# adalca/neurite

Measured on AMD Instinct MI355X. Metric: Mvoxels/sec interpn+Dice on 160^3 x 32-label, higher is better.
Workload: dtype f32

## Files before the change

neurite_amd/csrc/fused_wc.h:

```cpp

#pragma once

#include <type_traits>

#include "dice_reduce.h"
#include "interpn_core.h"

namespace {

#ifndef WC_NST_WARP
#define WC_NST_WARP 3
#endif
#ifndef WC_NST_FUSED
#define WC_NST_FUSED 2
#endif
#ifndef WC_NST_BWD
#define WC_NST_BWD 3
#endif
constexpr int WC_SLOTS = 128;
constexpr int WC_OVF = 16;
constexpr int WC_TRASH_ROW = WC_SLOTS + WC_OVF;
constexpr int WC_ROWS = WC_TRASH_ROW + 1;
constexpr unsigned WC_NOROW = 0x01ffffffu;
constexpr unsigned WC_TAGS_OFF = WC_ROWS * 128;
constexpr unsigned WC_LIST_OFF = WC_TAGS_OFF + 528;
constexpr unsigned WC_BC_OFF = WC_LIST_OFF + 512;
constexpr unsigned WC_WAVE_BYTES = WC_BC_OFF + 128;
constexpr unsigned WC_BLOCK_BYTES = 4 * WC_WAVE_BYTES;
static_assert(WC_LIST_OFF % 16 == 0 && WC_BC_OFF % 16 == 0 && WC_WAVE_BYTES % 16 == 0, "LDS layout");
static_assert((WC_SLOTS + 1) * 4 <= 528 && WC_ROWS <= 256, "LDS layout");
static_assert(2 * WC_BLOCK_BYTES <= 160 * 1024, "two blocks per CU");

typedef __attribute__((address_space(3))) char wc_lds_char;
typedef __attribute__((address_space(3))) nrt_f4 wc_lds_f4;
typedef __attribute__((address_space(3))) volatile nrt_i4 wc_lds_vi4;
typedef __attribute__((address_space(3))) volatile unsigned wc_lds_vu32;
typedef unsigned wc_u3 __attribute__((ext_vector_type(3)));
typedef unsigned wc_u4 __attribute__((ext_vector_type(4)));
typedef float wc_f3 __attribute__((ext_vector_type(3)));

__device__ __forceinline__ void wc_corner(float pv, float mx, int &i0, int &i1, float &w0) {
    const float cl = fminf(fmaxf(pv, 0.0f), mx);
    const float l0 = floorf(cl);
    const float l1 = fminf(nrt_add(l0, 1.0f), mx);
    i0 = (int)l0; i1 = (int)l1;
    w0 = nrt_sub(l1, cl);
}

__device__ __forceinline__ __amdgpu_buffer_rsrc_t wc_rsrc(const void *base, unsigned bytes) {
    const unsigned long long v = (unsigned long long)base;
    const void *u = (const void *)(((unsigned long long)(unsigned)__builtin_amdgcn_readfirstlane((unsigned)(v >> 32)) << 32) |
                                   (unsigned long long)(unsigned)__builtin_amdgcn_readfirstlane((unsigned)v));
    return __builtin_amdgcn_make_buffer_rsrc((void *)u, 0, __builtin_amdgcn_readfirstlane((int)bytes), 0x00020000);
}

struct WcBwd {
    const float *sums, *gdice;
    float eps;
    float *gloc;
};

template <int MODE, bool STORE, bool MM, bool FILL, bool DICE, int BWD = 0>
__device__ __forceinline__ void wc_item(const InterpArgs &a, const TileGeom &tg, const float *__restrict__ fixed, float *__restrict__ fpart,
                                        float *__restrict__ mpart, const XmWork &xw, char *wc_smem, const WcBwd &bw = WcBwd{nullptr, nullptr, 0.0f, nullptr}) {
    constexpr int G = 8, L = 32;
    static_assert(BWD == 0 || (DICE && !STORE && !MM), "the backward form reads a second row per voxel and stores the location gradient only");
    const int b = __builtin_amdgcn_readfirstlane(xw.b);
    const unsigned prow = (unsigned)__builtin_amdgcn_readfirstlane((int)xw.prow), ucol = (unsigned)__builtin_amdgcn_readfirstlane((int)xw.ucol);
    const unsigned RY = 1u << tg.lry, RZ = 1u << tg.lrz;
    const unsigned nRz = (tg.nTz + RZ - 1) / RZ;
    const unsigned reg = ucol / (RY * RZ), wr = ucol % (RY * RZ);
    const unsigned cy = (reg / nRz) * RY + wr / RZ, cz = (reg % nRz) * RZ + wr % RZ;
    const int x0 = __builtin_amdgcn_readfirstlane(xw.x0), y0 = (int)cy << 2, z0 = (int)cz << 3;
    int npass = __builtin_amdgcn_readfirstlane(xw.xlen);
    if (cy >= tg.nTy || cz >= tg.nTz || npass < 0) npass = 0;

    const int lane = threadIdx.x & 63, wave = threadIdx.x >> 6;
    const int g = lane >> 3, p = lane & 7;
    const int dzt = (0x1320 >> ((g & 3) * 4)) & 15;
    const int yy = y0 + 2 * (wave >> 1) + (g >> 2), zz = z0 + 4 * (wave & 1) + dzt;
    const bool yzvalid = (yy < a.O[1]) && (zz < a.O[2]);
    const int yc = min(yy, a.O[1] - 1), zc = min(zz, a.O[2] - 1);
    const unsigned qyz = (unsigned)yc * (unsigned)a.O[2] + (unsigned)zc, qstep = (unsigned)a.O[1] * (unsigned)a.O[2];
    const unsigned SY = (unsigned)a.S[1], SZ = (unsigned)a.S[2];
    const float mxx = (float)(a.S[0] - 1), mxy = (float)(a.S[1] - 1), mxz = (float)(a.S[2] - 1);
    const float fyc = (float)yc, fzc = (float)zc;
    const float ly = (yc == 0) ? 0.0f : ((yc == a.O[1] - 1) ? mxy : nrt_mul(a.delta[1], fyc));
    const float lz = (zc == 0) ? 0.0f : ((zc == a.O[2] - 1) ? mxz : nrt_mul(a.delta[2], fzc));

    const char *volb = (const char *)a.vol + (long long)b * a.vol_bs * 4ll;
    const unsigned long long volbytes = (unsigned long long)a.S[0] * SY * SZ * 128ull;
    const unsigned outbytes = a.nout * 128u;
    const __amdgpu_buffer_rsrc_t vres = wc_rsrc(volb, (unsigned)volbytes);
    const __amdgpu_buffer_rsrc_t lres = wc_rsrc(MODE != NRT_LOC_LINSPACE ? (const char *)(a.loc + (long long)b * a.loc_bs) : volb, a.nout * 12u);
    const __amdgpu_buffer_rsrc_t fres = wc_rsrc(DICE ? (const char *)fixed + (long long)b * a.out_bs * 4ll : volb, outbytes);
    const __amdgpu_buffer_rsrc_t ores = wc_rsrc(STORE ? (const char *)a.out + (long long)b * a.out_bs * 4ll : volb, outbytes);
    const __amdgpu_buffer_rsrc_t gres = wc_rsrc(BWD ? (const char *)(bw.gloc + (long long)b * a.nout * 3) : volb, a.nout * 12u);
    const unsigned gl_lane = (p == 0 && yzvalid) ? qyz * 12u : 0xffffffffu;
    float ca[4] = {0.0f, 0.0f, 0.0f, 0.0f}, cb[4] = {0.0f, 0.0f, 0.0f, 0.0f};
    if (BWD == 1) {
        const float *sm = bw.sums + (long long)b * 3 * L;
#pragma unroll
        for (int k = 0; k < 4; ++k) {
            const int l = p * 4 + k;
            const float num = 2.0f * sm[l] + bw.eps, den = sm[L + l] + sm[2 * L + l] + bw.eps;
            const float gd = bw.gdice[(long long)b * L + l];
            if (den != 0.0f) { ca[k] = 2.0f * gd / den; cb[k] = -2.0f * gd * num / (den * den); }
        }
    }
    const unsigned loc_lane = qyz * 12u, row_lane = (qyz * 8u + (unsigned)p) * 16u;
    const unsigned out_lane = yzvalid ? row_lane : 0xffffffffu;
    const unsigned loc_step = qstep * 12u, row_step = qstep * 128u;
    const unsigned p16 = (unsigned)p * 16u;

    wc_lds_char *wl = (wc_lds_char *)wc_smem + wave * WC_WAVE_BYTES;
    wc_lds_vu32 *tags = (wc_lds_vu32 *)(wl + WC_TAGS_OFF);
    wc_lds_char *lrow = wl + p * 16;
    tags[lane] = ~0u;
    tags[lane + 64] = ~0u;
    const bool cx1 = (p & 4) != 0, cy1 = (p & 2) != 0, cz1 = (p & 1) != 0;

    nrt_f2 stp_l = {0, 0}, stp_h = {0, 0}, stt_l = {0, 0}, stt_h = {0, 0}, spp_l = {0, 0}, spp_h = {0, 0};
    float mnt = INFINITY, mxt = -INFINITY, mnp = INFINITY, mxp = -INFINITY;

    struct Pass {
        float w0x, w0y, w0z;
        unsigned sl[8];
        unsigned lr[4], ld[4];
        unsigned xr[4], xd[4];
        int n;
        int xq;
        float mk[3];
        bool oob;
        nrt_f4 T;
        nrt_f4 F[4], Fx[4];
        float pn[3];
    };
    struct Mg { float w0x, w0y, w0z; bool oob, miss; unsigned rid, slot, t1, t2, mytag; float mk[3]; };
    constexpr int NST = ((BWD ? WC_NST_BWD : (DICE ? WC_NST_FUSED : WC_NST_WARP)) > 2) ? 3 : 2;
    constexpr bool XSH = NST == 3 && DICE;
    Pass A, B, C;
    nrt_f4 FxS[4] = {{0.f, 0.f, 0.f, 0.f}, {0.f, 0.f, 0.f, 0.f}, {0.f, 0.f, 0.f, 0.f}, {0.f, 0.f, 0.f, 0.f}};
    auto reset = [&](Pass &s) {
        s.w0x = s.w0y = s.w0z = 0.f; s.n = 0; s.xq = x0; s.oob = false; s.mk[0] = s.mk[1] = s.mk[2] = 0.f;
        s.T = (nrt_f4){0.f, 0.f, 0.f, 0.f};
#pragma unroll
        for (int i = 0; i < 4; ++i) { s.F[i] = s.Fx[i] = (nrt_f4){0.f, 0.f, 0.f, 0.f}; s.lr[i] = s.xr[i] = WC_NOROW << 7; s.ld[i] = s.xd[i] = WC_TRASH_ROW * 128u; }
#pragma unroll
        for (int i = 0; i < 8; ++i) s.sl[i] = 0;
        s.pn[0] = s.pn[1] = s.pn[2] = 0.f;
    };
    reset(A); reset(B);
    if (NST == 3) reset(C);

    auto fetch_loc = [&](int pass, Pass &s) {
        if (MODE != NRT_LOC_LINSPACE) {
            const wc_u3 v = __builtin_bit_cast(wc_u3, __builtin_amdgcn_raw_buffer_load_b96(lres, loc_lane, (unsigned)(x0 + pass) * loc_step, 0));
            s.pn[0] = __uint_as_float(v[0]); s.pn[1] = __uint_as_float(v[1]); s.pn[2] = __uint_as_float(v[2]);
        }
    };
    auto fetch_row = [&](unsigned rowoff) -> nrt_f4 {
        return __builtin_bit_cast(nrt_f4, __builtin_amdgcn_raw_buffer_load_b128(vres, rowoff | p16, 0, 0));
    };

    auto m1a = [&](int pass, const Pass &s, Mg &m) {
        const int xq = x0 + pass;
        float px, py, pz;
        if (MODE == NRT_LOC_ABSOLUTE) { px = s.pn[0]; py = s.pn[1]; pz = s.pn[2]; }
        else if (MODE == NRT_LOC_SHIFT) { px = nrt_add((float)xq, s.pn[0]); py = nrt_add(fyc, s.pn[1]); pz = nrt_add(fzc, s.pn[2]); }
        else { px = (xq == 0) ? 0.0f : ((xq == a.O[0] - 1) ? mxx : nrt_mul(a.delta[0], (float)xq)); py = ly; pz = lz; }
        int i0x, i1x, i0y, i1y, i0z, i1z;
        wc_corner(px, mxx, i0x, i1x, m.w0x);
        wc_corner(py, mxy, i0y, i1y, m.w0y);
        wc_corner(pz, mxz, i0z, i1z, m.w0z);
        m.oob = FILL ? ((px < 0.0f) || (px > mxx) || (py < 0.0f) || (py > mxy) || (pz < 0.0f) || (pz > mxz)) : false;
        if (BWD) {
            m.mk[0] = (fminf(fmaxf(px, 0.0f), mxx) == px) ? 1.0f : 0.0f;
            m.mk[1] = (fminf(fmaxf(py, 0.0f), mxy) == py) ? 1.0f : 0.0f;
            m.mk[2] = (fminf(fmaxf(pz, 0.0f), mxz) == pz) ? 1.0f : 0.0f;
        }
        const unsigned ix = cx1 ? i1x : i0x, iy = cy1 ? i1y : i0y, iz = cz1 ? i1z : i0z;
        m.rid = nrt_mad24(nrt_mad24(ix, SY, iy), SZ, iz);
        m.slot = ((ix & 3u) << 5) | ((iy & 3u) << 3) | (iz & 7u);
        m.mytag = (m.rid << 6) | (unsigned)lane;
        m.t1 = tags[m.slot];
    };
    auto m1b = [&](Mg &m) {
        m.miss = (m.t1 ^ m.mytag) >= 64u;
        tags[m.miss ? m.slot : (unsigned)WC_SLOTS] = m.mytag;
        m.t2 = tags[m.slot];
    };
    auto m1c = [&](int pass, const Mg &m, Pass &s) {
        const unsigned x2 = m.t2 ^ m.mytag;
        const bool served = x2 < 64u;
        const bool loader = m.miss && x2 == 0u;
        const bool orphan = !served;
        const unsigned long long Ml = __builtin_amdgcn_ballot_w64(loader), Mo = __builtin_amdgcn_ballot_w64(orphan);
        const unsigned long long Mf = Ml | Mo;
        const int no = __builtin_popcountll(Mo);
        int n = __builtin_popcountll(Mf);
        const unsigned ro = __builtin_amdgcn_mbcnt_hi((unsigned)(Mo >> 32), __builtin_amdgcn_mbcnt_lo((unsigned)Mo, 0u));
        const unsigned rf = __builtin_amdgcn_mbcnt_hi((unsigned)(Mf >> 32), __builtin_amdgcn_mbcnt_lo((unsigned)Mf, 0u));
        bool fetcher = loader || orphan;
        unsigned src = orphan ? (unsigned)WC_SLOTS + ro : m.slot;
        unsigned e = fetcher ? rf : (unsigned)n + ((unsigned)lane - rf);
        if (__builtin_expect(no > WC_OVF, 0)) {
            tags[lane] = ~0u;
            tags[lane + 64] = ~0u;
            e = (unsigned)lane; fetcher = true; src = (unsigned)lane; n = 64;
        }
        const unsigned src128 = src * 128u;
        const unsigned tp = ((e & 7u) << 3) | (e >> 3);
        typedef unsigned wc_u2 __attribute__((ext_vector_type(2)));
        *(__attribute__((address_space(3))) volatile wc_u2 *)(wl + WC_LIST_OFF + tp * 8u) =
            (wc_u2){fetcher ? (m.rid << 7) : (WC_NOROW << 7), fetcher ? src128 : (unsigned)WC_TRASH_ROW * 128u};
        ((__attribute__((address_space(3))) volatile unsigned short *)(wl + WC_BC_OFF))[lane] = (unsigned short)src128;
        const nrt_i4 la = *(wc_lds_vi4 *)(wl + WC_LIST_OFF + g * 64), lb = *(wc_lds_vi4 *)(wl + WC_LIST_OFF + g * 64 + 16);
        const nrt_i4 sh = *(wc_lds_vi4 *)(wl + WC_BC_OFF + g * 16);
        s.lr[0] = (unsigned)la[0]; s.ld[0] = (unsigned)la[1]; s.lr[1] = (unsigned)la[2]; s.ld[1] = (unsigned)la[3];
        s.lr[2] = (unsigned)lb[0]; s.ld[2] = (unsigned)lb[1]; s.lr[3] = (unsigned)lb[2]; s.ld[3] = (unsigned)lb[3];
        if (__builtin_expect(n > 32, 0)) {
            const nrt_i4 lc = *(wc_lds_vi4 *)(wl + WC_LIST_OFF + g * 64 + 32), le = *(wc_lds_vi4 *)(wl + WC_LIST_OFF + g * 64 + 48);
            s.xr[0] = (unsigned)lc[0]; s.xd[0] = (unsigned)lc[1]; s.xr[1] = (unsigned)lc[2]; s.xd[1] = (unsigned)lc[3];
            s.xr[2] = (unsigned)le[0]; s.xd[2] = (unsigned)le[1]; s.xr[3] = (unsigned)le[2]; s.xd[3] = (unsigned)le[3];
        }
#pragma unroll
        for (int c = 0; c < 4; ++c) { s.sl[2 * c] = (unsigned)sh[c] & 0xffffu; s.sl[2 * c + 1] = (unsigned)sh[c] >> 16; }
        s.w0x = m.w0x; s.w0y = m.w0y; s.w0z = m.w0z; s.oob = m.oob; s.n = n;
        if (BWD) { s.mk[0] = m.mk[0]; s.mk[1] = m.mk[1]; s.mk[2] = m.mk[2]; }
        s.xq = x0 + pass;
    };
    auto issue = [&](Pass &s) {
#pragma unroll
        for (int i = 0; i < 4; ++i) s.F[i] = fetch_row(s.lr[i]);
        if (!XSH && __builtin_expect(s.n > 32, 0)) {
#pragma unroll
            for (int i = 0; i < 4; ++i) s.Fx[i] = fetch_row(s.xr[i]);
        }
        if (DICE) s.T = __builtin_bit_cast(nrt_f4, __builtin_amdgcn_raw_buffer_load_b128(fres, row_lane, (unsigned)s.xq * row_step, 2));
    };
    auto issue_x = [&](Pass &s) {
        if (XSH && __builtin_expect(s.n > 32, 0)) {
#pragma unroll
            for (int i = 0; i < 4; ++i) FxS[i] = fetch_row(s.xr[i]);
        }
    };
    auto deliver = [&](Pass &s) {
#pragma unroll
        for (int i = 0; i < 4; ++i) *(wc_lds_f4 *)(lrow + s.ld[i]) = s.F[i];
        if (__builtin_expect(s.n > 32, 0)) {
#pragma unroll
            for (int i = 0; i < 4; ++i) *(wc_lds_f4 *)(lrow + s.xd[i]) = XSH ? FxS[i] : s.Fx[i];
        }
    };

    const int last = npass - 1;
    auto step = [&](int pass, Pass &s, Pass &o, Pass &nx, auto masked) {
        constexpr bool MASKED = decltype(masked)::value;
        issue(o);
        __builtin_amdgcn_sched_barrier(0);
        deliver(s);
        nrt_f4 R[8];
#pragma unroll
        for (int corner = 0; corner < 8; ++corner) R[corner] = *(const wc_lds_f4 *)(lrow + s.sl[corner]);
        __builtin_amdgcn_sched_barrier(0);
        Mg m;
        m1a(min(pass + NST, last), s, m);
        __builtin_amdgcn_sched_barrier(0);
        const float w1x = nrt_sub(1.0f, s.w0x), w1y = nrt_sub(1.0f, s.w0y), w1z = nrt_sub(1.0f, s.w0z);
        const nrt_f2 wy2 = {s.w0y, w1y}, wz2 = {s.w0z, w1z};
        const nrt_f2 wxy0 = (nrt_f2){s.w0x, s.w0x} * wy2, wxy1 = (nrt_f2){w1x, w1x} * wy2;
        nrt_f2 wt2[4];
        wt2[0] = (nrt_f2){wxy0[0], wxy0[0]} * wz2;
        wt2[1] = (nrt_f2){wxy0[1], wxy0[1]} * wz2;
        wt2[2] = (nrt_f2){wxy1[0], wxy1[0]} * wz2;
        wt2[3] = (nrt_f2){wxy1[1], wxy1[1]} * wz2;
        nrt_f2 al = {0.0f, 0.0f}, ah = {0.0f, 0.0f};
        constexpr bool BLEND = BWD != 2;
#pragma unroll
        for (int corner = 0; corner < (BLEND ? 4 : 0); ++corner) {
            const float wt = wt2[corner >> 1][corner & 1];
            const nrt_f2 w2 = {wt, wt};
            al = al + w2 * (nrt_f2){R[corner][0], R[corner][1]};
            ah = ah + w2 * (nrt_f2){R[corner][2], R[corner][3]};
        }
        asm volatile("" : "+v"(al), "+v"(ah));
        __builtin_amdgcn_sched_barrier(0);
        m1b(m);
        __builtin_amdgcn_sched_barrier(0);
#pragma unroll
        for (int corner = 4; corner < (BLEND ? 8 : 4); ++corner) {
            const float wt = wt2[corner >> 1][corner & 1];
            const nrt_f2 w2 = {wt, wt};
            al = al + w2 * (nrt_f2){R[corner][0], R[corner][1]};
            ah = ah + w2 * (nrt_f2){R[corner][2], R[corner][3]};
        }
        nrt_f4 acc = {al[0], al[1], ah[0], ah[1]};
        const unsigned xqcur = (unsigned)s.xq;
        const float cw0x = s.w0x, cw0y = s.w0y, cw0z = s.w0z, cmx = s.mk[0], cmy = s.mk[1], cmz = s.mk[2];
        const bool coob = s.oob;
        if (!BWD) {
            if (FILL) {
#pragma unroll
                for (int c = 0; c < 4; ++c) acc[c] = apply_fill(acc[c], s.oob, a.fill_f);
            }
            if (STORE) __builtin_amdgcn_raw_buffer_store_b128(__builtin_bit_cast(wc_u4, acc), ores, out_lane, (unsigned)s.xq * row_step, 2);
        }
        const nrt_f4 Tcur = s.T;
        asm volatile("" : "+v"(acc));
        __builtin_amdgcn_sched_barrier(0);
        m1c(min(pass + NST, last), m, s);
        __builtin_amdgcn_sched_barrier(0);
        if (BWD) {
            nrt_f2 gl2 = {Tcur[0], Tcur[1]}, gh2 = {Tcur[2], Tcur[3]};
            if (BWD == 1) {
                gl2 = __builtin_elementwise_fma((nrt_f2){cb[0], cb[1]}, (nrt_f2){acc[0], acc[1]}, (nrt_f2){ca[0], ca[1]} * gl2);
                gh2 = __builtin_elementwise_fma((nrt_f2){cb[2], cb[3]}, (nrt_f2){acc[2], acc[3]}, (nrt_f2){ca[2], ca[3]} * gh2);
            }
            if (FILL && coob) { gl2 = (nrt_f2){0.0f, 0.0f}; gh2 = gl2; }
            float gacc[3];
            loc_grad_rows(R, gl2, gh2, cw0x, w1x, cw0y, w1y, cw0z, w1z, cmx, cmy, cmz, gacc);
#pragma unroll
            for (int d = 0; d < 3; ++d) {
                float r = gacc[d];
                r += __int_as_float(__builtin_amdgcn_update_dpp(0, __float_as_int(r), 0xB1, 0xF, 0xF, true));
                r += __int_as_float(__builtin_amdgcn_update_dpp(0, __float_as_int(r), 0x4E, 0xF, 0xF, true));
                r += __int_as_float(__builtin_amdgcn_update_dpp(0, __float_as_int(r), 0x141, 0xF, 0xF, true));
                gacc[d] = r;
            }
            __builtin_amdgcn_raw_buffer_store_b96(__builtin_bit_cast(wc_u3, (wc_f3){gacc[0], gacc[1], gacc[2]}), gres, gl_lane, xqcur * loc_step, 0);
        } else if (DICE) {
            nrt_f4 T = Tcur;
            if (MASKED) {
#pragma unroll
                for (int c = 0; c < 4; ++c) { T[c] = yzvalid ? T[c] : 0.0f; acc[c] = yzvalid ? acc[c] : 0.0f; }
            }
            const nrt_f2 pl = {acc[0], acc[1]}, ph = {acc[2], acc[3]}, tl = {T[0], T[1]}, th = {T[2], T[3]};
            stp_l = stp_l + tl * pl; stp_h = stp_h + th * ph;
            stt_l = stt_l + tl * tl; stt_h = stt_h + th * th;
            spp_l = spp_l + pl * pl; spp_h = spp_h + ph * ph;
            if (MM) {
                if (!MASKED || yzvalid) {
#pragma unroll
                    for (int c = 0; c < 4; ++c) {
                        mnt = fminf(mnt, Tcur[c]); mxt = fmaxf(mxt, Tcur[c]);
                        mnp = fminf(mnp, acc[c]); mxp = fmaxf(mxp, acc[c]);
                    }
                }
            }
        }
        if (DICE && !BWD) asm volatile("" : "+v"(stp_l), "+v"(stp_h), "+v"(stt_l), "+v"(stt_h), "+v"(spp_l), "+v"(spp_h));
        else asm volatile("" :: "v"(acc));
        __builtin_amdgcn_sched_barrier(0);
        fetch_loc(min(pass + 2 * NST, last), s);
        issue_x(nx);
        __builtin_amdgcn_sched_barrier(0);
    };
    auto march = [&](auto masked) {
        Mg m;
        if constexpr (NST == 3) {
            fetch_loc(0, A);
            fetch_loc(min(1, last), B);
            fetch_loc(min(2, last), C);
            m1a(0, A, m); m1b(m); m1c(0, m, A);
            issue(A);
            fetch_loc(min(3, last), A);
            m1a(min(1, last), B, m); m1b(m); m1c(min(1, last), m, B);
            issue(B);
            fetch_loc(min(4, last), B);
            m1a(min(2, last), C, m); m1b(m); m1c(min(2, last), m, C);
            fetch_loc(min(5, last), C);
            issue_x(A);
            __builtin_amdgcn_sched_barrier(0);
            int pass = 0;
            for (; pass + 2 < npass; pass += 3) {
                step(pass, A, C, B, masked);
                step(pass + 1, B, A, C, masked);
                step(pass + 2, C, B, A, masked);
            }
            if (pass < npass) step(pass, A, C, B, masked);
            if (pass + 1 < npass) step(pass + 1, B, A, C, masked);
            return;
        }
        fetch_loc(0, A);
        fetch_loc(min(1, last), B);
        m1a(0, A, m); m1b(m); m1c(0, m, A);
        issue(A);
        fetch_loc(min(2, last), A);
        m1a(min(1, last), B, m); m1b(m); m1c(min(1, last), m, B);
        fetch_loc(min(3, last), B);
        __builtin_amdgcn_sched_barrier(0);
        int pass = 0;
        for (; pass + 1 < npass; pass += 2) {
            step(pass, A, B, B, masked);
            step(pass + 1, B, A, A, masked);
        }
        if (pass < npass) step(pass, A, B, B, masked);
    };
    if (npass > 0) {
        if (DICE && !BWD && __builtin_amdgcn_ballot_w64(!yzvalid) != 0ull) march(std::true_type());
        else march(std::false_type());
    }

    if (!DICE || BWD) return;
    nrt_f4 stp = {stp_l[0], stp_l[1], stp_h[0], stp_h[1]}, stt = {stt_l[0], stt_l[1], stt_h[0], stt_h[1]},
           spp = {spp_l[0], spp_l[1], spp_h[0], spp_h[1]};
#pragma unroll
    for (int c = 0; c < 4; ++c) {
        stp[c] = wave_xor_add(stp[c], G);
        stt[c] = wave_xor_add(stt[c], G);
        spp[c] = wave_xor_add(spp[c], G);
    }
    for (int off = 1; off < NRT_WAVE; off <<= 1) {
        mnt = fminf(mnt, __shfl_xor(mnt, off, NRT_WAVE)); mxt = fmaxf(mxt, __shfl_xor(mxt, off, NRT_WAVE));
        mnp = fminf(mnp, __shfl_xor(mnp, off, NRT_WAVE)); mxp = fmaxf(mxp, __shfl_xor(mxp, off, NRT_WAVE));
    }
    __syncthreads();
    float (*red)[3 * L + 4] = (float (*)[3 * L + 4])wc_smem;
    if (lane < G) {
#pragma unroll
        for (int c = 0; c < 4; ++c) {
            red[wave][0 * L + 4 * lane + c] = stp[c];
            red[wave][1 * L + 4 * lane + c] = stt[c];
            red[wave][2 * L + 4 * lane + c] = spp[c];
        }
    }
    if (lane == 0) { red[wave][3 * L + 0] = mnt; red[wave][3 * L + 1] = mxt; red[wave][3 * L + 2] = mnp; red[wave][3 * L + 3] = mxp; }
    __syncthreads();
    const long long pbase = (long long)b * tg.prows + prow;
    for (int i = threadIdx.x; i < 3 * L; i += 256) {
        float s = red[0][i];
#pragma unroll
        for (int w2 = 1; w2 < 4; ++w2) s += red[w2][i];
        fpart[pbase * 3 * L + i] = s;
    }
    if (threadIdx.x < 4) {
        float m = red[0][3 * L + threadIdx.x];
        for (int w2 = 1; w2 < 4; ++w2)
            m = (threadIdx.x & 1) ? fmaxf(m, red[w2][3 * L + threadIdx.x]) : fminf(m, red[w2][3 * L + threadIdx.x]);
        mpart[pbase * 4 + threadIdx.x] = m;
    }
    xmarch_zero_rows(tg, xw, 3 * L, fpart, mpart);
}


template <typename ITEM>
__device__ __forceinline__ void wc_persistent_loop(const TileGeom &tg, int O0, unsigned *__restrict__ queue, ITEM item) {
    __shared__ unsigned s_next[2];
    const unsigned home = blockIdx.x % NRT_NXCD;
    for (;;) {
        __syncthreads();
        if (threadIdx.x == 0) {
            unsigned kk = home, jb = 0xffffffffu;
            for (unsigned t = 0; t < NRT_NXCD; ++t) {
                const unsigned q = (home + t) % NRT_NXCD;
                const unsigned v = atomicAdd(&queue[q * 16u], 1u);
                if (v < tg.items_x) { kk = q; jb = v; break; }
            }
            s_next[0] = kk; s_next[1] = jb;
        }
        __syncthreads();
        const unsigned kk = s_next[0], jb = s_next[1];
        if (jb == 0xffffffffu) break;
        XmWork xw;
        if (!xmarch_work_at(tg, O0, kk, jb, xw)) continue;
        item(xw);
    }
    if (threadIdx.x == 0 && atomicAdd(&queue[NRT_NXCD * 16u], 1u) == gridDim.x - 1) {
        for (unsigned q = 0; q <= NRT_NXCD; ++q) queue[q * 16u] = 0u;
    }
}

template <int MODE, bool STORE, bool MM, bool FILL, bool DICE = true, bool PERSIST = false>
__global__ __launch_bounds__(256, 2) void warp_dice_wc(InterpArgs a, TileGeom tg, const float *__restrict__ fixed,
                                                        float *__restrict__ fpart, float *__restrict__ mpart, unsigned *__restrict__ queue) {
    extern __shared__ __attribute__((aligned(16))) char wc_smem[];
    if (!PERSIST) {
        XmWork xw;
        if (!xmarch_work(tg, a.O[0], xw)) return;
        wc_item<MODE, STORE, MM, FILL, DICE>(a, tg, fixed, fpart, mpart, xw, wc_smem);
        return;
    }
    wc_persistent_loop(tg, a.O[0], queue, [&](const XmWork &xw) { wc_item<MODE, STORE, MM, FILL, DICE>(a, tg, fixed, fpart, mpart, xw, wc_smem); });
}

template <int MODE, bool FILL, int BWD, bool PERSIST>
__global__ __launch_bounds__(256, 2) void warp_dice_wc_bwd(InterpArgs a, TileGeom tg, const float *__restrict__ rows, WcBwd bw,
                                                            unsigned *__restrict__ queue) {
    extern __shared__ __attribute__((aligned(16))) char wc_smem[];
    if (!PERSIST) {
        XmWork xw;
        if (!xmarch_work(tg, a.O[0], xw)) return;
        wc_item<MODE, false, false, FILL, true, BWD>(a, tg, rows, nullptr, nullptr, xw, wc_smem, bw);
        return;
    }
    wc_persistent_loop(tg, a.O[0], queue, [&](const XmWork &xw) { wc_item<MODE, false, false, FILL, true, BWD>(a, tg, rows, nullptr, nullptr, xw, wc_smem, bw); });
}

inline bool wc_persistent(const TileGeom &tg) { return NRT_NXCD * tg.items_x > 2u * (unsigned)nrt_num_cus(); }
static_assert(NRT_RING_GATHER_OFF == 0 && (NRT_NXCD + 1) * 16 <= NRT_RING_CCE_OFF, "the work counters of a launch stay in the gather's words of a slot");

template <int MODE, bool STORE, bool MM, bool FILL>
int launch_wc_inst(const InterpArgs &a, const TileGeom &tg, unsigned nblocks, int batch, const float *fixed, float *fpart, float *mpart,
                   hipStream_t st) {
    const unsigned items = NRT_NXCD * tg.items_x, slots = 2u * (unsigned)nrt_num_cus();
    unsigned *queue = wc_persistent(tg) ? nrt_ring_slot(st) : nullptr;
    if (queue) {
        if (hipFuncSetAttribute((const void *)warp_dice_wc<MODE, STORE, MM, FILL, true, true>, hipFuncAttributeMaxDynamicSharedMemorySize,
                                (int)WC_BLOCK_BYTES) != hipSuccess)
            return NRT_ERR_LAUNCH;
        hipLaunchKernelGGL((warp_dice_wc<MODE, STORE, MM, FILL, true, true>), dim3(nrt_xcd_grid(slots)), dim3(256), WC_BLOCK_BYTES, st, a, tg, fixed,
                           fpart, mpart, queue);
        return NRT_OK;
    }
    if (hipFuncSetAttribute((const void *)warp_dice_wc<MODE, STORE, MM, FILL>, hipFuncAttributeMaxDynamicSharedMemorySize, (int)WC_BLOCK_BYTES) != hipSuccess)
        return NRT_ERR_LAUNCH;
    hipLaunchKernelGGL((warp_dice_wc<MODE, STORE, MM, FILL>), dim3(items), dim3(256), WC_BLOCK_BYTES, st, a, tg, fixed, fpart, mpart,
                       (unsigned *)nullptr);
    (void)nblocks; (void)batch;
    return NRT_OK;
}

template <int MODE, bool FILL>
int launch_wc_fill(const InterpArgs &a, const TileGeom &tg, unsigned nblocks, int batch, bool store, bool minmax, const float *fixed,
                   float *fpart, float *mpart, hipStream_t st) {
    if (store) return minmax ? launch_wc_inst<MODE, true, true, FILL>(a, tg, nblocks, batch, fixed, fpart, mpart, st)
                             : launch_wc_inst<MODE, true, false, FILL>(a, tg, nblocks, batch, fixed, fpart, mpart, st);
    return minmax ? launch_wc_inst<MODE, false, true, FILL>(a, tg, nblocks, batch, fixed, fpart, mpart, st)
                  : launch_wc_inst<MODE, false, false, FILL>(a, tg, nblocks, batch, fixed, fpart, mpart, st);
}

template <int MODE>
int launch_wc_mode(const InterpArgs &a, const TileGeom &tg, unsigned nblocks, int batch, bool store, bool minmax, const float *fixed,
                   float *fpart, float *mpart, hipStream_t st) {
    return a.has_fill ? launch_wc_fill<MODE, true>(a, tg, nblocks, batch, store, minmax, fixed, fpart, mpart, st)
                      : launch_wc_fill<MODE, false>(a, tg, nblocks, batch, store, minmax, fixed, fpart, mpart, st);
}

inline bool wc_applies(const TileGeom &tg, int G, const InterpArgs &a) {
    return tg.x_march && G == 8 && tg.lty == 2 && tg.ltz == 3 && !tg.plane_major &&
           (unsigned long long)a.S[0] * a.S[1] * a.S[2] * 128ull < 0xffffff00ull;
}

inline int launch_wc(const InterpArgs &a, const TileGeom &tg, unsigned nblocks, int batch, int mode, bool store, bool minmax,
                     const float *fixed, float *fpart, float *mpart, hipStream_t st) {
    switch (mode) {
        case NRT_LOC_ABSOLUTE: return launch_wc_mode<NRT_LOC_ABSOLUTE>(a, tg, nblocks, batch, store, minmax, fixed, fpart, mpart, st);
        case NRT_LOC_SHIFT: return launch_wc_mode<NRT_LOC_SHIFT>(a, tg, nblocks, batch, store, minmax, fixed, fpart, mpart, st);
        default: return launch_wc_mode<NRT_LOC_LINSPACE>(a, tg, nblocks, batch, store, minmax, fixed, fpart, mpart, st);
    }
}

template <int MODE, bool FILL>
int launch_wc_interpn_inst(const InterpArgs &a, const TileGeom &tg, hipStream_t st) {
    const unsigned items = NRT_NXCD * tg.items_x, slots = 2u * (unsigned)nrt_num_cus();
    unsigned *queue = (items > slots) ? nrt_ring_slot(st) : nullptr;
    if (queue) {
        if (hipFuncSetAttribute((const void *)warp_dice_wc<MODE, true, false, FILL, false, true>, hipFuncAttributeMaxDynamicSharedMemorySize,
                                (int)WC_BLOCK_BYTES) != hipSuccess)
            return NRT_ERR_LAUNCH;
        hipLaunchKernelGGL((warp_dice_wc<MODE, true, false, FILL, false, true>), dim3(nrt_xcd_grid(slots)), dim3(256), WC_BLOCK_BYTES, st, a, tg,
                           (const float *)nullptr, (float *)nullptr, (float *)nullptr, queue);
        return NRT_OK;
    }
    if (hipFuncSetAttribute((const void *)warp_dice_wc<MODE, true, false, FILL, false>, hipFuncAttributeMaxDynamicSharedMemorySize,
                            (int)WC_BLOCK_BYTES) != hipSuccess)
        return NRT_ERR_LAUNCH;
    hipLaunchKernelGGL((warp_dice_wc<MODE, true, false, FILL, false>), dim3(items), dim3(256), WC_BLOCK_BYTES, st, a, tg, (const float *)nullptr,
                       (float *)nullptr, (float *)nullptr, (unsigned *)nullptr);
    return NRT_OK;
}

template <int MODE, bool FILL, int BWD>
int launch_wc_bwd_inst(const InterpArgs &a, const TileGeom &tg, const float *rows, const WcBwd &bw, hipStream_t st) {
    const unsigned items = NRT_NXCD * tg.items_x, slots = 2u * (unsigned)nrt_num_cus();
    unsigned *queue = (items > slots) ? nrt_ring_slot(st) : nullptr;
    if (queue) {
        if (hipFuncSetAttribute((const void *)warp_dice_wc_bwd<MODE, FILL, BWD, true>, hipFuncAttributeMaxDynamicSharedMemorySize, (int)WC_BLOCK_BYTES) != hipSuccess)
            return NRT_ERR_LAUNCH;
        hipLaunchKernelGGL((warp_dice_wc_bwd<MODE, FILL, BWD, true>), dim3(nrt_xcd_grid(slots)), dim3(256), WC_BLOCK_BYTES, st, a, tg, rows, bw, queue);
        return NRT_OK;
    }
    if (hipFuncSetAttribute((const void *)warp_dice_wc_bwd<MODE, FILL, BWD, false>, hipFuncAttributeMaxDynamicSharedMemorySize, (int)WC_BLOCK_BYTES) != hipSuccess)
        return NRT_ERR_LAUNCH;
    hipLaunchKernelGGL((warp_dice_wc_bwd<MODE, FILL, BWD, false>), dim3(items), dim3(256), WC_BLOCK_BYTES, st, a, tg, rows, bw, (unsigned *)nullptr);
    return NRT_OK;
}

template <int MODE, bool FILL>
int launch_wc_bwd_mode(const InterpArgs &a, const TileGeom &tg, const float *rows, const WcBwd &bw, hipStream_t st) {
    return bw.sums ? launch_wc_bwd_inst<MODE, FILL, 1>(a, tg, rows, bw, st) : launch_wc_bwd_inst<MODE, FILL, 2>(a, tg, rows, bw, st);
}

}

int nrt_wc_bwd_launch(const void *args, int batch, int mode, const float *rows, const float *sums, const float *grad_dice, float eps,
                      float *grad_loc, void *stream) {
    const InterpArgs &a = *(const InterpArgs *)args;
    if (mode != NRT_LOC_ABSOLUTE && mode != NRT_LOC_SHIFT) return NRT_ERR_INVALID_ARG;
    TileGeom tg;
    unsigned nblocks, grid;
    const int t = xmarch_default_tune();
    tile_geometry(a.O, 8, t, t, tg, nblocks);
    xmarch_setup_mixed(a.O, batch, t, tg, grid);
    hipStream_t st = nrt_stream(stream);
    const WcBwd bw = {sums, grad_dice, eps, grad_loc};
    int rc;
    if (mode == NRT_LOC_ABSOLUTE) rc = a.has_fill ? launch_wc_bwd_mode<NRT_LOC_ABSOLUTE, true>(a, tg, rows, bw, st) : launch_wc_bwd_mode<NRT_LOC_ABSOLUTE, false>(a, tg, rows, bw, st);
    else rc = a.has_fill ? launch_wc_bwd_mode<NRT_LOC_SHIFT, true>(a, tg, rows, bw, st) : launch_wc_bwd_mode<NRT_LOC_SHIFT, false>(a, tg, rows, bw, st);
    if (rc != NRT_OK) return rc;
    NRT_CHECK_LAUNCH();
    return NRT_OK;
}

bool nrt_wc_interpn_supported(const void *args, int batch) {
    const InterpArgs &a = *(const InterpArgs *)args;
    if (a.C != 32 || !xmarch_applies(a.O, batch)) return false;
    if ((unsigned long long)a.nout * 128ull >= (1ull << 32)) return false;
    if ((long long)a.S[0] * a.S[1] >= (1 << 24) || a.S[2] >= (1 << 24) || (long long)a.O[0] * a.O[1] >= (1 << 24) || a.O[2] >= (1 << 24)) return false;
    TileGeom tg;
    unsigned nblocks, grid;
    const int t = xmarch_default_tune();
    tile_geometry(a.O, 8, t, t, tg, nblocks);
    xmarch_setup_mixed(a.O, batch, t, tg, grid);
    return wc_applies(tg, 8, a);
}

int nrt_wc_interpn_launch(const void *args, int batch, int mode, void *stream) {
    const InterpArgs &a = *(const InterpArgs *)args;
    TileGeom tg;
    unsigned nblocks, grid;
    const int t = xmarch_default_tune();
    tile_geometry(a.O, 8, t, t, tg, nblocks);
    xmarch_setup_mixed(a.O, batch, t, tg, grid);
    hipStream_t st = nrt_stream(stream);
    int rc;
    switch (mode) {
        case NRT_LOC_ABSOLUTE: rc = a.has_fill ? launch_wc_interpn_inst<NRT_LOC_ABSOLUTE, true>(a, tg, st) : launch_wc_interpn_inst<NRT_LOC_ABSOLUTE, false>(a, tg, st); break;
        case NRT_LOC_SHIFT: rc = a.has_fill ? launch_wc_interpn_inst<NRT_LOC_SHIFT, true>(a, tg, st) : launch_wc_interpn_inst<NRT_LOC_SHIFT, false>(a, tg, st); break;
        default: rc = a.has_fill ? launch_wc_interpn_inst<NRT_LOC_LINSPACE, true>(a, tg, st) : launch_wc_interpn_inst<NRT_LOC_LINSPACE, false>(a, tg, st); break;
    }
    if (rc != NRT_OK) return rc;
    NRT_CHECK_LAUNCH();
    return NRT_OK;
}
```

Before: 19770.

## Shrink always-fetched row groups to three and skip unused row stores

Makes the number of always-issued row fetch groups configurable (default still 4). Row fetches and LDS deliveries beyond the live count are skipped using a wave-uniform count, taken with readfirstlane. The first loop iteration is peeled out of the three-stage and two-stage march loops. The aim is to cut wasted LDS writes and fetches when few unique rows are needed and to give the scheduler a steady-state loop, at the cost of extra branching and larger code.

```diff
diff --git a/neurite_amd/csrc/fused_wc.h b/neurite_amd/csrc/fused_wc.h
--- a/neurite_amd/csrc/fused_wc.h
+++ b/neurite_amd/csrc/fused_wc.h
@@ -16,6 +16,9 @@
 #endif
 #ifndef WC_NST_BWD
 #define WC_NST_BWD 3
+#endif
+#ifndef WC_FIXED_GROUPS
+#define WC_FIXED_GROUPS 4
 #endif
 constexpr int WC_SLOTS = 128;
 constexpr int WC_OVF = 16;
@@ -123,29 +126,35 @@
     nrt_f2 stp_l = {0, 0}, stp_h = {0, 0}, stt_l = {0, 0}, stt_h = {0, 0}, spp_l = {0, 0}, spp_h = {0, 0};
     float mnt = INFINITY, mxt = -INFINITY, mnp = INFINITY, mxp = -INFINITY;
 
+    constexpr int FG = WC_FIXED_GROUPS, NX = 8 - FG;
+    static_assert(FG == 3 || FG == 4, "WC_FIXED_GROUPS");
     struct Pass {
         float w0x, w0y, w0z;
         unsigned sl[8];
-        unsigned lr[4], ld[4];
-        unsigned xr[4], xd[4];
+        unsigned lr[FG], ld[FG];
+        unsigned xr[NX], xd[NX];
         int n;
         int xq;
         float mk[3];
         bool oob;
         nrt_f4 T;
-        nrt_f4 F[4], Fx[4];
+        nrt_f4 F[FG], Fx[NX];
         float pn[3];
     };
     struct Mg { float w0x, w0y, w0z; bool oob, miss; unsigned rid, slot, t1, t2, mytag; float mk[3]; };
     constexpr int NST = ((BWD ? WC_NST_BWD : (DICE ? WC_NST_FUSED : WC_NST_WARP)) > 2) ? 3 : 2;
     constexpr bool XSH = NST == 3 && DICE;
     Pass A, B, C;
-    nrt_f4 FxS[4] = {{0.f, 0.f, 0.f, 0.f}, {0.f, 0.f, 0.f, 0.f}, {0.f, 0.f, 0.f, 0.f}, {0.f, 0.f, 0.f, 0.f}};
+    nrt_f4 FxS[NX];
+#pragma unroll
+    for (int i = 0; i < NX; ++i) FxS[i] = (nrt_f4){0.f, 0.f, 0.f, 0.f};
     auto reset = [&](Pass &s) {
         s.w0x = s.w0y = s.w0z = 0.f; s.n = 0; s.xq = x0; s.oob = false; s.mk[0] = s.mk[1] = s.mk[2] = 0.f;
         s.T = (nrt_f4){0.f, 0.f, 0.f, 0.f};
 #pragma unroll
-        for (int i = 0; i < 4; ++i) { s.F[i] = s.Fx[i] = (nrt_f4){0.f, 0.f, 0.f, 0.f}; s.lr[i] = s.xr[i] = WC_NOROW << 7; s.ld[i] = s.xd[i] = WC_TRASH_ROW * 128u; }
+        for (int i = 0; i < FG; ++i) { s.F[i] = (nrt_f4){0.f, 0.f, 0.f, 0.f}; s.lr[i] = WC_NOROW << 7; s.ld[i] = WC_TRASH_ROW * 128u; }
+#pragma unroll
+        for (int i = 0; i < NX; ++i) { s.Fx[i] = (nrt_f4){0.f, 0.f, 0.f, 0.f}; s.xr[i] = WC_NOROW << 7; s.xd[i] = WC_TRASH_ROW * 128u; }
 #pragma unroll
         for (int i = 0; i < 8; ++i) s.sl[i] = 0;
         s.pn[0] = s.pn[1] = s.pn[2] = 0.f;
@@ -218,39 +227,47 @@
         const nrt_i4 la = *(wc_lds_vi4 *)(wl + WC_LIST_OFF + g * 64), lb = *(wc_lds_vi4 *)(wl + WC_LIST_OFF + g * 64 + 16);
         const nrt_i4 sh = *(wc_lds_vi4 *)(wl + WC_BC_OFF + g * 16);
         s.lr[0] = (unsigned)la[0]; s.ld[0] = (unsigned)la[1]; s.lr[1] = (unsigned)la[2]; s.ld[1] = (unsigned)la[3];
-        s.lr[2] = (unsigned)lb[0]; s.ld[2] = (unsigned)lb[1]; s.lr[3] = (unsigned)lb[2]; s.ld[3] = (unsigned)lb[3];
+        s.lr[2] = (unsigned)lb[0]; s.ld[2] = (unsigned)lb[1];
+        if (FG == 4) { s.lr[FG - 1] = (unsigned)lb[2]; s.ld[FG - 1] = (unsigned)lb[3]; }
+        else { s.xr[0] = (unsigned)lb[2]; s.xd[0] = (unsigned)lb[3]; }
         if (__builtin_expect(n > 32, 0)) {
             const nrt_i4 lc = *(wc_lds_vi4 *)(wl + WC_LIST_OFF + g * 64 + 32), le = *(wc_lds_vi4 *)(wl + WC_LIST_OFF + g * 64 + 48);
-            s.xr[0] = (unsigned)lc[0]; s.xd[0] = (unsigned)lc[1]; s.xr[1] = (unsigned)lc[2]; s.xd[1] = (unsigned)lc[3];
-            s.xr[2] = (unsigned)le[0]; s.xd[2] = (unsigned)le[1]; s.xr[3] = (unsigned)le[2]; s.xd[3] = (unsigned)le[3];
+            s.xr[NX - 4] = (unsigned)lc[0]; s.xd[NX - 4] = (unsigned)lc[1]; s.xr[NX - 3] = (unsigned)lc[2]; s.xd[NX - 3] = (unsigned)lc[3];
+            s.xr[NX - 2] = (unsigned)le[0]; s.xd[NX - 2] = (unsigned)le[1]; s.xr[NX - 1] = (unsigned)le[2]; s.xd[NX - 1] = (unsigned)le[3];
         }
 #pragma unroll
         for (int c = 0; c < 4; ++c) { s.sl[2 * c] = (unsigned)sh[c] & 0xffffu; s.sl[2 * c + 1] = (unsigned)sh[c] >> 16; }
-        s.w0x = m.w0x; s.w0y = m.w0y; s.w0z = m.w0z; s.oob = m.oob; s.n = n;
+        s.w0x = m.w0x; s.w0y = m.w0y; s.w0z = m.w0z; s.oob = m.oob;
+        s.n = __builtin_amdgcn_readfirstlane(n);
         if (BWD) { s.mk[0] = m.mk[0]; s.mk[1] = m.mk[1]; s.mk[2] = m.mk[2]; }
         s.xq = x0 + pass;
     };
     auto issue = [&](Pass &s) {
 #pragma unroll
-        for (int i = 0; i < 4; ++i) s.F[i] = fetch_row(s.lr[i]);
-        if (!XSH && __builtin_expect(s.n > 32, 0)) {
-#pragma unroll
-            for (int i = 0; i < 4; ++i) s.Fx[i] = fetch_row(s.xr[i]);
+        for (int i = 0; i < FG; ++i) s.F[i] = fetch_row(s.lr[i]);
+        if (!XSH && __builtin_expect(s.n > 8 * FG, 0)) {
+#pragma unroll
+            for (int i = 0; i < NX; ++i)
+                if (i == 0 || s.n > 8 * (FG + i)) s.Fx[i] = fetch_row(s.xr[i]);
         }
         if (DICE) s.T = __builtin_bit_cast(nrt_f4, __builtin_amdgcn_raw_buffer_load_b128(fres, row_lane, (unsigned)s.xq * row_step, 2));
     };
     auto issue_x = [&](Pass &s) {
-        if (XSH && __builtin_expect(s.n > 32, 0)) {
-#pragma unroll
-            for (int i = 0; i < 4; ++i) FxS[i] = fetch_row(s.xr[i]);
+        if (XSH && __builtin_expect(s.n > 8 * FG, 0)) {
+#pragma unroll
+            for (int i = 0; i < NX; ++i)
+                if (i == 0 || s.n > 8 * (FG + i)) FxS[i] = fetch_row(s.xr[i]);
         }
     };
     auto deliver = [&](Pass &s) {
-#pragma unroll
-        for (int i = 0; i < 4; ++i) *(wc_lds_f4 *)(lrow + s.ld[i]) = s.F[i];
-        if (__builtin_expect(s.n > 32, 0)) {
-#pragma unroll
-            for (int i = 0; i < 4; ++i) *(wc_lds_f4 *)(lrow + s.xd[i]) = XSH ? FxS[i] : s.Fx[i];
+        *(wc_lds_f4 *)(lrow + s.ld[0]) = s.F[0];
+#pragma unroll
+        for (int i = 1; i < FG; ++i)
+            if (s.n > 8 * i) *(wc_lds_f4 *)(lrow + s.ld[i]) = s.F[i];
+        if (__builtin_expect(s.n > 8 * FG, 0)) {
+#pragma unroll
+            for (int i = 0; i < NX; ++i)
+                if (i == 0 || s.n > 8 * (FG + i)) *(wc_lds_f4 *)(lrow + s.xd[i]) = XSH ? FxS[i] : s.Fx[i];
         }
     };
 
@@ -373,10 +390,15 @@
             issue_x(A);
             __builtin_amdgcn_sched_barrier(0);
             int pass = 0;
-            for (; pass + 2 < npass; pass += 3) {
-                step(pass, A, C, B, masked);
-                step(pass + 1, B, A, C, masked);
-                step(pass + 2, C, B, A, masked);
+            if (npass >= 3) {
+                step(0, A, C, B, masked);
+                step(1, B, A, C, masked);
+                step(2, C, B, A, masked);
+                for (pass = 3; pass + 2 < npass; pass += 3) {
+                    step(pass, A, C, B, masked);
+                    step(pass + 1, B, A, C, masked);
+                    step(pass + 2, C, B, A, masked);
+                }
             }
             if (pass < npass) step(pass, A, C, B, masked);
             if (pass + 1 < npass) step(pass + 1, B, A, C, masked);
@@ -391,9 +413,13 @@
         fetch_loc(min(3, last), B);
         __builtin_amdgcn_sched_barrier(0);
         int pass = 0;
-        for (; pass + 1 < npass; pass += 2) {
-            step(pass, A, B, B, masked);
-            step(pass + 1, B, A, A, masked);
+        if (npass >= 2) {
+            step(0, A, B, B, masked);
+            step(1, B, A, A, masked);
+            for (pass = 2; pass + 1 < npass; pass += 2) {
+                step(pass, A, B, B, masked);
+                step(pass + 1, B, A, A, masked);
+            }
         }
         if (pass < npass) step(pass, A, B, B, masked);
     };
```

After: 21000, median of 6. +6.2%, better.
